# bergmanlab/TELR

Measured on AMD Instinct MI355X. Metric: gbp_aligned_per_s, higher is better.
Workload: dtype int16

## Files before the change

telr_amd/csrc/kernels.hip.h:

```cpp
#pragma once
#include <hip/hip_runtime.h>
#include <stdint.h>

#define TELR_NEG      (-(1 << 28))
#include "part_plan.h"
#define SK_TILE       1024
#define SK_THREADS    256
#define DP_DMAX       4096

struct ChainOpt {
    int32_t max_gap, bw, min_cnt, min_chain_score, chain_gap_q8, chain_skip_q8;
    int32_t dense_n, dense_span, mw_n;
};
struct DpOpt {
    int32_t a, b, q, e, q2, e2, sc_ambi, zdrop;
    int32_t cx_scale, cx_open, cx_emax, cx_emin, cx_dec, cx_flat;
};
__host__ __device__ __forceinline__ int d_cx_ext(const DpOpt &o, int len) { int v = o.cx_emax - o.cx_dec * len; return v > o.cx_emin ? v : o.cx_emin; }
__host__ __device__ __forceinline__ int d_cx_cost(const DpOpt &o, int L)
{
    int t = o.cx_open;
    for (int i = 0; i < L && i < o.cx_flat; ++i) t += d_cx_ext(o, i);
    if (L > o.cx_flat) t += (L - o.cx_flat) * o.cx_emin;
    return t;
// ... 1332 lines not shown
        for (int h = 1; h < R - 1; ++h) Ms = hfull[h] > Ms ? hfull[h] : Ms;
        Ms += (int32_t)sp1 + 1;
        const int inext = j0 + 64 + lane;
        const uint64_t knext = inext < n ? a[inext] : 0;
        const uint32_t ng = (uint32_t)(knext >> 32), nqp = (uint32_t)A_Q(knext), nsp1 = (uint32_t)A_SPAN(knext) - 1u;
        const int32_t nB = 2 * A_SPAN(knext) + 1;
        int32_t myB = 0, myp = -1;
        const int jn = n - j0 < 64 ? n - j0 : 64;
        for (int jj = 0; jj < jn; ++jj) {
            const int j = j0 + jj;
            const uint32_t gj = gcur, gj1 = gj + 1u;
            const uint32_t gnext = jj < 63 ? (uint32_t)__builtin_amdgcn_readlane((int)gi, jj + 1) : (uint32_t)__builtin_amdgcn_readlane((int)ng, 0);
            gcur = gnext;
            int32_t sB = __builtin_amdgcn_readlane(B, jj);
            const int32_t sMs = __builtin_amdgcn_readlane(Ms, jj);
            const bool me = lane == jj;
            if (sMs > (sB >> 1)) {
                const uint32_t gfar = jj ? (uint32_t)__builtin_amdgcn_readlane((int)hg[0], jj - 1) : (uint32_t)__builtin_amdgcn_readlane((int)hg[1], 63);
                if (gj - gfar <= max_gap) {
                    const uint32_t qS = (uint32_t)__builtin_amdgcn_readlane((int)qi, jj), spS = (uint32_t)__builtin_amdgcn_readlane((int)sp1, jj);
                    int32_t Bl = NEG * 2, bl = -1;
#pragma unroll
                    for (int h = R - 1; h >= 0; --h) {
                        const bool in_set = h == 0 ? lane < jj : h == R - 1 ? lane >= jj : true;
                        int32_t Bt = Bl, bt = bl;
                        d_chain_push<SKIP>(gj, qS, spS, hg[h] + 1u, hq[h] + 1u, hf[h], j0 - 64 * (h + 1) + lane, max_gap, ddc, gap_q8, skip_q8, Bt, bt);
                        Bl = in_set ? Bt : Bl; bl = in_set ? bt : bl;
                    }
                    int32_t m = Bl;
#pragma unroll
                    for (int s = 32; s >= 1; s >>= 1) { const int32_t v = __shfl_xor(m, s); m = v > m ? v : m; }
                    if (m > sB) {
                        int32_t w = Bl == m ? bl : -1;
#pragma unroll
                        for (int s = 32; s >= 1; s >>= 1) { const int32_t v = __shfl_xor(w, s); w = v > w ? v : w; }
                        B = me ? m : B; bp = me ? w : bp; sB = __builtin_amdgcn_readfirstlane(m);
                    }
                }
            }
            const uint32_t qj1 = (uint32_t)__builtin_amdgcn_readlane((int)qi, jj) + 1u;
            {
                const uint64_t one = 1ULL << jj; uint64_t sv;
                asm volatile("s_mov_b64 %[sv], exec\n\ts_mov_b64 exec, %[m]\n\t"
                             "v_mov_b32 %[myB], %[B]\n\tv_mov_b32 %[myp], %[bp]\n\tv_mov_b32 %[gi], %[ng]\n\tv_mov_b32 %[sp1], %[nsp1]\n\t"
                             "v_mov_b32 %[qi], %[nqp]\n\tv_mov_b32 %[B], %[nB]\n\ts_mov_b64 exec, %[sv]"
                             : [myB] "+v"(myB), [myp] "+v"(myp), [gi] "+v"(gi), [sp1] "+v"(sp1), [qi] "+v"(qi), [B] "+v"(B), [sv] "=&s"(sv)
                             : [bp] "v"(bp), [ng] "v"(ng), [nsp1] "v"(nsp1), [nqp] "v"(nqp), [nB] "v"(nB), [m] "s"(one));
            }
            if (gnext - gj <= max_gap) {
                const int32_t fj2p2 = (sB & ~1) + 2;
                d_chain_push<SKIP>(gi, qi, sp1, gj1, qj1, fj2p2, j, max_gap, ddc, gap_q8, skip_q8, B, bp);
            }
        }
        if (lane < jn) { f[base + j0 + lane] = myB >> 1; p[base + j0 + lane] = (myB & 1) ? -1 : myp + pdelta; }
        if (j0 + 64 < n) {
#pragma unroll
            for (int h = R - 1; h >= 1; --h) { hg[h] = hg[h - 1]; hq[h] = hq[h - 1]; hf[h] = hf[h - 1]; hsuf[h] = hsuf[h - 1]; hfull[h] = hfull[h - 1]; }
            const uint64_t k = a[j0 + lane];
            hg[0] = (uint32_t)(k >> 32); hq[0] = (uint32_t)A_Q(k); hf[0] = (myB & ~1) + 2;
            const int32_t fv = myB >> 1;
            int32_t inc = fv, suf = fv;
#pragma unroll
            for (int s = 1; s < 64; s <<= 1) {
                const int32_t u = __shfl_up(inc, s), d = __shfl_down(suf, s);
                if (lane >= s) inc = u > inc ? u : inc;
                if (lane + s < 64) suf = d > suf ? d : suf;
            }
            const int32_t ex = __shfl_up(inc, 1);
            pre0 = lane ? ex : NEG; hsuf[0] = suf; hfull[0] = __builtin_amdgcn_readlane(suf, 0);
        }
    }
}

__device__ __forceinline__ bool d_chain_dense(const uint64_t *__restrict__ a, const int n, const ChainOpt &o)
{
    if (o.dense_n <= 0 || n < o.dense_n || n < 128) return false;
    const int i = (int)(((int64_t)(threadIdx.x & 63) * (n - 65)) / 63);
    const uint32_t g0 = (uint32_t)(a[i] >> 32), g1 = (uint32_t)(a[i + 64] >> 32);
    return __popcll(__ballot(g1 - g0 <= (uint32_t)o.dense_span)) >= 21;
}
template <int R, bool SKIP>
__device__ __forceinline__ void d_chain_run_mw(const uint64_t *__restrict__ keys, const int64_t base, const int n, const int pdelta,
                                               const ChainOpt &o, int32_t *__restrict__ f, int32_t *__restrict__ p, uint4 *ring, int32_t *done_s)
{
    static_assert(R >= 2, "one wave is the push loop");
    constexpr int RING = 64 * R;
    const int lane = threadIdx.x & 63, wv = __builtin_amdgcn_readfirstlane((int)(threadIdx.x >> 6));
    const uint64_t *a = keys + base;
    const uint32_t max_gap = (uint32_t)o.max_gap, ddc = o.bw < o.max_gap ? (uint32_t)(o.max_gap - 1 - o.bw) : 0u;
    const uint32_t gap_q8 = (uint32_t)o.chain_gap_q8, skip_q8 = (uint32_t)o.chain_skip_q8;
    if (threadIdx.x == 0) *done_s = 0;
    __syncthreads();
    const int nchunk = (n + 63) >> 6;
    uint32_t gi, qi, sp1; int32_t B, bp = -1;
    { const int i = wv * 64 + lane; const uint64_t k = i < n ? a[i] : 0; gi = (uint32_t)(k >> 32); qi = (uint32_t)A_Q(k); sp1 = (uint32_t)A_SPAN(k) - 1u; B = 2 * A_SPAN(k) + 1; }
    for (int c = wv; c < nchunk; c += R) {
        const int j0 = c * 64;
        const int inext = j0 + RING + lane;
        const uint64_t knext = inext < n ? a[inext] : 0;
        const uint32_t ng = (uint32_t)(knext >> 32), nqp = (uint32_t)A_Q(knext), nsp1 = (uint32_t)A_SPAN(knext) - 1u;
        const int32_t nB = 2 * A_SPAN(knext) + 1;
        int j = j0 - 64 * (R - 1); if (j < 0) j = 0;
        int polls = 0;
        while (j < j0) {
            const int avail = __builtin_amdgcn_readfirstlane(__hip_atomic_load(done_s, __ATOMIC_ACQUIRE, __HIP_MEMORY_SCOPE_WORKGROUP));
            if (avail <= j) { if (++polls > (1 << 24)) break; __builtin_amdgcn_s_sleep(2); continue; }
            int lim = avail < j0 ? avail : j0; if (lim > j + 64) lim = j + 64;
            const int cnt = lim - j;
            uint4 e = make_uint4(0u, 0u, 0u, 0u);
            if (lane < cnt) e = ring[(j + lane) & (RING - 1)];
            for (int t = 0; t < cnt; ++t) {
                const uint32_t gj1 = (uint32_t)__builtin_amdgcn_readlane((int)e.x, t), qj1 = (uint32_t)__builtin_amdgcn_readlane((int)e.y, t);
                const int32_t fj2p2 = __builtin_amdgcn_readlane((int)e.z, t);
                d_chain_push<SKIP>(gi, qi, sp1, gj1, qj1, fj2p2, j + t, max_gap, ddc, gap_q8, skip_q8, B, bp);
            }
            j = lim;
        }
        const int jn = n - j0 < 64 ? n - j0 : 64;
        int32_t myB = 0, myp = -1; uint32_t myg = 0, myq = 0;
        for (int jj = 0; jj < jn; ++jj) {
            const uint32_t gj1 = (uint32_t)__builtin_amdgcn_readlane((int)gi, jj) + 1u, qj1 = (uint32_t)__builtin_amdgcn_readlane((int)qi, jj) + 1u;
            const int32_t fj2p2 = (__builtin_amdgcn_readlane(B, jj) & ~1) + 2;
            {
                const uint64_t one = 1ULL << jj; uint64_t sv;
                asm volatile("s_mov_b64 %[sv], exec\n\ts_mov_b64 exec, %[m]\n\t"
                             "v_mov_b32 %[myB], %[B]\n\tv_mov_b32 %[myp], %[bp]\n\tv_mov_b32 %[myg], %[gi]\n\tv_mov_b32 %[myq], %[qi]\n\t"
                             "v_mov_b32 %[gi], %[ng]\n\tv_mov_b32 %[qi], %[nqp]\n\tv_mov_b32 %[sp1], %[nsp1]\n\tv_mov_b32 %[B], %[nB]\n\ts_mov_b64 exec, %[sv]"
                             : [myB] "+v"(myB), [myp] "+v"(myp), [myg] "+v"(myg), [myq] "+v"(myq), [gi] "+v"(gi), [qi] "+v"(qi), [sp1] "+v"(sp1), [B] "+v"(B), [sv] "=&s"(sv)
                             : [bp] "v"(bp), [ng] "v"(ng), [nqp] "v"(nqp), [nsp1] "v"(nsp1), [nB] "v"(nB), [m] "s"(one));
            }
            d_chain_push<SKIP>(gi, qi, sp1, gj1, qj1, fj2p2, j0 + jj, max_gap, ddc, gap_q8, skip_q8, B, bp);
            if ((jj & 7) == 7 || jj == jn - 1) {
                if (lane >= (jj & ~7) && lane <= jj) ring[(j0 + lane) & (RING - 1)] = make_uint4(myg + 1u, myq + 1u, (uint32_t)((myB & ~1) + 2), 0u);
                __hip_atomic_store(done_s, j0 + jj + 1, __ATOMIC_RELEASE, __HIP_MEMORY_SCOPE_WORKGROUP);
            }
        }
        if (lane < jn) { f[base + j0 + lane] = myB >> 1; p[base + j0 + lane] = (myB & 1) ? -1 : myp + pdelta; }
    }
}
__device__ __forceinline__ bool d_chain_is_mw(const bool dense, const int n, const ChainOpt &o) { return dense && o.mw_n > 0 && n >= o.mw_n; }
template <int R, bool SKIP, int MODE>
__device__ __forceinline__ void d_chain_any(const uint64_t *__restrict__ keys, const int64_t base, const int n, const int pdelta,
                                            const ChainOpt &o, int32_t *__restrict__ f, int32_t *__restrict__ p, const bool skip_mw)
{
    if constexpr (MODE == 0 || R < 2) d_chain_run<R, SKIP>(keys, base, n, pdelta, o, f, p);
    else if constexpr (MODE == 1) d_chain_run_lazy<R, SKIP>(keys, base, n, pdelta, o, f, p);
    else {
        const bool dense = d_chain_dense(keys + base, n, o);
        if (skip_mw && d_chain_is_mw(dense, n, o)) return;
        if (dense) d_chain_run<R, SKIP>(keys, base, n, pdelta, o, f, p);
        else d_chain_run_lazy<R, SKIP>(keys, base, n, pdelta, o, f, p);
    }
}
template <int R, bool SKIP, int MODE = 2>
__global__ void __launch_bounds__(64) k_chain(const uint64_t *__restrict__ keys, const int32_t *__restrict__ q_aoff, int32_t nq,
                                              ChainOpt o, int32_t *__restrict__ f, int32_t *__restrict__ p, const int32_t *__restrict__ q_order, int32_t skip_mw)
{
    if ((int)blockIdx.x >= nq) return;
    const int q = q_order ? q_order[blockIdx.x] : blockIdx.x;
    d_chain_any<R, SKIP, MODE>(keys, q_aoff[q], q_aoff[q + 1] - q_aoff[q], 0, o, f, p, skip_mw != 0);
}
template <int R, bool SKIP>
__global__ void __launch_bounds__(64 * R) k_chain_mw(const uint64_t *__restrict__ keys, const int32_t *__restrict__ q_aoff, int32_t nq, const int32_t *__restrict__ list,
                                                     ChainOpt o, int32_t *__restrict__ f, int32_t *__restrict__ p)
{
    __shared__ uint4 ring[64 * R];
    __shared__ int32_t done_s;
    if ((int)blockIdx.x >= nq) return;
    const int q = list ? list[blockIdx.x] : (int)blockIdx.x;
    const int64_t base = q_aoff[q]; const int n = q_aoff[q + 1] - q_aoff[q];
    if (!d_chain_is_mw(d_chain_dense(keys + base, n, o), n, o)) return;
    d_chain_run_mw<R, SKIP>(keys, base, n, 0, o, f, p, ring, &done_s);
}
#define CHAIN_ISL_NQ 4096
__global__ void __launch_bounds__(256) k_isl_heads(const uint64_t *__restrict__ keys, const int32_t *__restrict__ q_aoff, int32_t nq, uint32_t max_gap, int32_t *__restrict__ head)
{
    const int q = blockIdx.x;
    if (q >= nq) return;
    const int64_t base = q_aoff[q]; const int n = q_aoff[q + 1] - q_aoff[q];
    for (int i = threadIdx.x; i < n; i += blockDim.x)
        head[base + i] = i == 0 || (uint32_t)(keys[base + i] >> 32) - (uint32_t)(keys[base + i - 1] >> 32) > max_gap;
}
__global__ void __launch_bounds__(256) k_isl_fill(const int32_t *__restrict__ q_aoff, int32_t nq, const int32_t *__restrict__ head, const int32_t *__restrict__ rank, int32_t na,
                                                  int32_t *__restrict__ isl_off, int32_t *__restrict__ isl_pd)
{
    const int q = blockIdx.x;
    if (q >= nq) return;
    const int64_t base = q_aoff[q]; const int n = q_aoff[q + 1] - q_aoff[q];
    for (int i = threadIdx.x; i < n; i += blockDim.x) if (head[base + i]) { const int id = rank[base + i]; isl_off[id] = (int32_t)base + i; isl_pd[id] = i; }
    if (q == 0 && threadIdx.x == 0) isl_off[rank[na]] = na;
}
template <int R, bool SKIP, int MODE = 2>
__global__ void __launch_bounds__(64) k_chain_isl(const uint64_t *__restrict__ keys, const int32_t *__restrict__ isl_off, const int32_t *__restrict__ isl_pd, const int32_t *__restrict__ nisl,
                                                  ChainOpt o, int32_t *__restrict__ f, int32_t *__restrict__ p)
{
    const int n_isl = *nisl;
    for (int s = blockIdx.x; s < n_isl; s += gridDim.x)
        d_chain_any<R, SKIP, MODE>(keys, isl_off[s], isl_off[s + 1] - isl_off[s], isl_pd[s], o, f, p, false);
}

#define CHAIN_SCAN_H    5000
#define CHAIN_SCAN_SKIP 25
__device__ __forceinline__ uint32_t d_wave_scan_max0(uint32_t v)
{
    v = max(v, (uint32_t)__builtin_amdgcn_update_dpp(0, (int)v, 0x111, 0xf, 0xf, true));
    v = max(v, (uint32_t)__builtin_amdgcn_update_dpp(0, (int)v, 0x112, 0xf, 0xf, true));
    v = max(v, (uint32_t)__builtin_amdgcn_update_dpp(0, (int)v, 0x114, 0xf, 0xf, true));
    v = max(v, (uint32_t)__builtin_amdgcn_update_dpp(0, (int)v, 0x118, 0xf, 0xf, true));
    v = max(v, (uint32_t)__builtin_amdgcn_update_dpp(0, (int)v, 0x142, 0xa, 0xf, true));
    v = max(v, (uint32_t)__builtin_amdgcn_update_dpp(0, (int)v, 0x143, 0xc, 0xf, true));
    return v;
}
template <bool SKIP>
__device__ __forceinline__ void d_chain_run_scan(const uint64_t *__restrict__ keys, const int64_t base, const int n, const int pdelta,
                                                 const ChainOpt &o, int32_t *__restrict__ f, int32_t *__restrict__ p, int32_t *__restrict__ mark,
                                                 uint8_t *__restrict__ fl)
{
    const int lane = threadIdx.x & 63;
    const uint64_t *a = keys + base;
    const uint32_t max_gap = (uint32_t)o.max_gap, ddc = o.bw < o.max_gap ? (uint32_t)(o.max_gap - 1 - o.bw) : 0u;
    const uint32_t gap_q8 = (uint32_t)o.chain_gap_q8, skip_q8 = (uint32_t)o.chain_skip_q8;
    uint32_t wg = 0, wq = 0; int32_t wf = 0, wp = -1;
    uint64_t kb = lane < n ? a[lane] : 0;
    for (int i0 = 0; i0 < n; i0 += 64) {
        const uint64_t kn = i0 + 64 + lane < n ? a[i0 + 64 + lane] : 0;
        const int m = n - i0 < 64 ? n - i0 : 64;
        int32_t of = 0, op = -1;
        for (int ii = 0; ii < m; ++ii) {
            const int i = i0 + ii;
            const uint32_t gi = (uint32_t)__builtin_amdgcn_readlane((int)(uint32_t)(kb >> 32), ii);
            const uint32_t klo = (uint32_t)__builtin_amdgcn_readlane((int)(uint32_t)kb, ii);
            const uint32_t qi = (klo >> 8) & 0xffffffu, sp = klo & 0xffu;
            const int32_t gpos = (int32_t)(gi & 0x7fffffffu);
            const int lo = i - CHAIN_SCAN_H > 0 ? i - CHAIN_SCAN_H : 0;
            int32_t best = (int32_t)sp, bp = -1, nskip = 0;
            for (int c = 0; ; ++c) {
                const int jt = i - 1 - 64 * c, j = jt - lane;
                if (jt < lo) break;
                uint32_t g = wg, q = wq; int32_t fj2p2 = wf, pj = wp; bool mk = false;
                if (c > 0 && j >= lo) {
                    const uint64_t k = a[j];
                    g = (uint32_t)(k >> 32); q = (uint32_t)A_Q(k);
                    fj2p2 = 2 * f[base + j] + 2;
                    const int32_t pa = p[base + j];
                    pj = pa >= 0 ? pa - pdelta : -1;
                    mk = mark[base + j] == (int32_t)(base + i);
                }
                const bool inw = j >= lo && ((g ^ gi) >> 31) == 0u && gpos - (int32_t)(g & 0x7fffffffu) <= (int32_t)max_gap;
                bool ok;
                const int32_t v2 = d_chain_link<SKIP>(gi, qi, sp - 1u, g + 1u, q + 1u, fj2p2, max_gap, ddc, gap_q8, skip_q8, ok);
                const bool valid = inw && ok;
                const int32_t v = v2 >> 1;
                const uint32_t u = valid && v > best ? (uint32_t)(v - best) : 0u;
                const uint32_t pre = d_wave_scan_max0(u);
                const uint32_t ex = (uint32_t)__shfl_up((int)pre, 1);
                const bool imp = u > (lane ? ex : 0u);
                fl[lane] = 0;
                const int tl = jt - pj;
                if (valid && pj >= 0 && tl < 64) fl[tl] = 1;
                __builtin_amdgcn_fence(__ATOMIC_SEQ_CST, "wavefront");
                mk = mk || fl[lane] != 0;
                __builtin_amdgcn_fence(__ATOMIC_SEQ_CST, "wavefront");
                const int32_t s = valid ? (imp ? -1 : (mk ? 1 : 0)) : 0;
                const int32_t T = nskip + (int32_t)d_wave_scan_add((uint32_t)s);
                const int32_t x = T + (int32_t)d_wave_scan_max0(T < 0 ? (uint32_t)(-T) : 0u);
                const uint64_t brk = __ballot(x > CHAIN_SCAN_SKIP);
                const int b = brk ? __ffsll((unsigned long long)brk) - 1 : 64;
                const uint64_t scanned = b == 64 ? ~0ULL : ((1ULL << b) - 1);
                const uint64_t im = __ballot(imp) & scanned;
                if (im) {
                    const int hl = 63 - __clzll((long long)im);
                    best += (int32_t)__builtin_amdgcn_readlane((int)u, hl);
                    bp = jt - hl;
                }
                const uint64_t win = __ballot(inw);
                const bool more = b == 64 && win == ~0ULL && jt - 64 >= lo;
                if (!more) break;
                if (valid && pj >= 0 && tl >= 64) mark[base + pj] = (int32_t)(base + i);
                nskip = __builtin_amdgcn_readlane(x, 63);
                __threadfence_block();
            }
            of = lane == ii ? best : of; op = lane == ii ? bp : op;
            wg = (uint32_t)__shfl_up((int)wg, 1); wq = (uint32_t)__shfl_up((int)wq, 1); wf = __shfl_up(wf, 1); wp = __shfl_up(wp, 1);
            if (lane == 0) { wg = gi; wq = qi; wf = 2 * best + 2; wp = bp; }
        }
        if (lane < m) {
            f[base + i0 + lane] = of; p[base + i0 + lane] = op >= 0 ? op + pdelta : -1;
            mark[base + i0 + lane] = -1;
        }
        __threadfence_block();
        kb = kn;
    }
}
template <bool SKIP>
__global__ void __launch_bounds__(64) k_chain_scan(const uint64_t *__restrict__ keys, const int32_t *__restrict__ q_aoff, int32_t nq,
                                                   ChainOpt o, int32_t *__restrict__ f, int32_t *__restrict__ p, int32_t *__restrict__ mark,
                                                   const int32_t *__restrict__ q_order)
{
    __shared__ uint8_t fl[64];
    if ((int)blockIdx.x >= nq) return;
    const int q = q_order ? q_order[blockIdx.x] : blockIdx.x;
    d_chain_run_scan<SKIP>(keys, q_aoff[q], q_aoff[q + 1] - q_aoff[q], 0, o, f, p, mark, fl);
}
template <bool SKIP>
__global__ void __launch_bounds__(64) k_chain_scan_isl(const uint64_t *__restrict__ keys, const int32_t *__restrict__ isl_off, const int32_t *__restrict__ isl_pd,
                                                       const int32_t *__restrict__ nisl, ChainOpt o, int32_t *__restrict__ f, int32_t *__restrict__ p,
                                                       int32_t *__restrict__ mark)
{
    __shared__ uint8_t fl[64];
    const int n_isl = *nisl;
    for (int s = blockIdx.x; s < n_isl; s += gridDim.x)
        d_chain_run_scan<SKIP>(keys, isl_off[s], isl_off[s + 1] - isl_off[s], isl_pd[s], o, f, p, mark, fl);
}
// ... 2148 lines not shown
```

telr_amd/csrc/telr_engine.hip:

```cpp
#include <hip/hip_runtime.h>
#include <cstring>
#include <string.h>
#include <rocprim/rocprim.hpp>
#include <algorithm>
#include <atomic>
#include <immintrin.h>
#include <chrono>
#include <cmath>
#include <condition_variable>
#include <cstdio>
#include <cstdlib>
#include <cstring>
#include <map>
#include <memory>
#include <mutex>
#include <string>
#include <thread>
#include <sys/mman.h>
#include <vector>
#include "../../include/telr_hip.h"
#include "kernels.hip.h"
#include "range_plan.h"
#include "sam_records.h"
#define TELR_HAVE_SEED_ARGS 1
// ... 1344 lines not shown
        hipLaunchKernelGGL(k_tb_scatter, dim3(np / 256 + 1), dim3(256), 0, st, d_probs, d_clslist, np, coff, d_tboff);
        HIPCHK(hipGetLastError());
        HIPCHK(hipMemcpyAsync(&tb_total, d_tboff + np, 8, hipMemcpyDeviceToHost, st));
        HIPCHK(hipStreamSynchronize(st));
    }
    uint8_t *d_tb;
    TRY(ctx_buf_t(ctx, ("tb" + sfx).c_str(), (size_t)tb_total + 256, &d_tb));
    if (primary) TRY(ctx_buf_t(ctx, "rawcig", (size_t)cg_total + 16, d_rawcig_io));
    DpArgs D; D.qseq2 = qs->d_seq2; D.qnmask = qs->d_nmask; D.tseq2 = tg->d_seq2; D.tnmask = tg->d_nmask; D.probs = d_probs;
    D.qtot = qs->padded_bases; D.ttot = tg->padded_bases;
    D.o.a = mo->a; D.o.b = mo->b; D.o.q = mo->q; D.o.e = mo->e; D.o.q2 = mo->q2; D.o.e2 = mo->e2; D.o.sc_ambi = mo->sc_ambi; D.o.zdrop = mo->zdrop;
    D.o.cx_scale = D.o.cx_open = D.o.cx_emax = D.o.cx_emin = D.o.cx_dec = D.o.cx_flat = 0;
    if (mo->cx_scale > 0) {
        const int S = mo->cx_scale;
        D.o.a *= S; D.o.b *= S; D.o.sc_ambi *= S; D.o.zdrop *= S;
        D.o.cx_scale = S; D.o.cx_open = mo->cx_open; D.o.cx_emax = mo->cx_ext_max; D.o.cx_emin = mo->cx_ext_min; D.o.cx_dec = mo->cx_decay;
        D.o.cx_flat = mo->cx_decay > 0 && mo->cx_ext_max > mo->cx_ext_min ? (mo->cx_ext_max - mo->cx_ext_min + mo->cx_decay - 1) / mo->cx_decay : 0;
    }
    D.tb = d_tb; D.cig = *d_rawcig_io; D.res = d_res; D.dcap = 0;
    D.retry = d_retry; D.tb4 = L.tb4_mask; D.tag8_steps = L.tag8_steps;
    static const bool tb_split = !ab_on("tb_one_launch");
    int nw = 0; uint32_t *d_wv2 = nullptr;
    {
        PkPlan plan; plan.woff[0] = 0;
        for (int c = 0; c < PK_NC; ++c) { const int ppw = 64 / DP_CLASS[PK_CLS(c)].lpp; plan.woff[c + 1] = plan.woff[c] + (h_cls[PK_CLS(c)] + ppw - 1) / ppw; }
        nw = plan.woff[PK_NC];
        if (nw > 0) {
            uint32_t *d_wk, *d_wv, *d_wk2;
            TRY(ctx_buf_t(ctx, ("pk_wkey" + sfx).c_str(), (size_t)nw, &d_wk));
            TRY(ctx_buf_t(ctx, ("pk_wval" + sfx).c_str(), (size_t)nw, &d_wv));
            TRY(ctx_buf_t(ctx, ("pk_wkey2" + sfx).c_str(), (size_t)nw, &d_wk2));
            TRY(ctx_buf_t(ctx, ("pk_wval2" + sfx).c_str(), (size_t)nw, &d_wv2));
            hipLaunchKernelGGL(k_pk_waves, dim3((nw + 255) / 256), dim3(256), 0, st, d_probs, d_clslist, coff, plan, d_wk, d_wv);
            HIPCHK(hipGetLastError());
            size_t tbytes = 0;
            HIPCHK(rocprim::radix_sort_pairs_desc(nullptr, tbytes, d_wk, d_wk2, d_wv, d_wv2, (size_t)nw, 0, 16, st));
            void *tmp; TRY(ctx_buf(ctx, "rp_tmp", tbytes, &tmp));
            HIPCHK(rocprim::radix_sort_pairs_desc(tmp, tbytes, d_wk, d_wk2, d_wv, d_wv2, (size_t)nw, 0, 16, st));
        }
    }
    HIPCHK(hipEventRecord(ctx->ev_fork, st));
    int side = 0;
    std::vector<hipStream_t> used;
    static const bool serial = getenv("TELR_SERIAL") != nullptr;
    auto side_stream = [&]() { if (serial) return st; hipStream_t s2 = ctx->side[side % TELR_NSIDE]; ++side; used.push_back(s2); return s2; };
    auto launch = [&](int c, DpKernel kernel, hipStream_t s2) -> int {
        const int nl = h_cls[c];
        int threads = DP_CLASS[c].lpp > 64 ? DP_CLASS[c].lpp : 64, ppb = DP_CLASS[c].lpp < 64 ? 64 / DP_CLASS[c].lpp : 1;
        size_t lds = 0;
        D.list = d_clslist + coff.off[c]; D.nlist = nl; D.dcap = 0;
        if (DP_CLASS[c].family == DPF_LDS) {
            D.dcap = DP_CLASS[c].maxd;
            lds = (size_t)(D.dcap + 2) * 5 * 4;
            static const bool one_wave = ab_on("dp_one_wave");
            if (one_wave) { kernel = k_dp; threads = 64; }
            if (lds > 48 * 1024) HIPCHK(hipFuncSetAttribute((const void*)kernel, hipFuncAttributeMaxDynamicSharedMemorySize, (int)lds));
        }
        if (c == CLS_PKX64 && nl < 8192) { kernel = k_dp_pkx16; ppb = 4; }
        hipLaunchKernelGGL(kernel, dim3((nl + ppb - 1) / ppb), dim3(threads), lds, s2, D);
        HIPCHK(hipGetLastError());
        return TELR_OK;
    };
    for (const SideLaunch &row : SIDE_LAUNCH) {
        const int c = row.cls, nl = h_cls[c];
        if (nl == 0) continue;
        hipStream_t s2 = side_stream();
        HIPCHK(hipStreamWaitEvent(s2, ctx->ev_fork, 0));
        TRY(launch(c, row.kernel, s2));
        if (tb_split) {
            const int tbw_max = 2048;
            if (row.lane_walk || nl > tbw_max) hipLaunchKernelGGL(k_traceback, dim3((nl + 63) / 64), dim3(64), 0, s2, d_probs, d_res, nl, d_tb, *d_rawcig_io, d_retry, D.list);
            else hipLaunchKernelGGL(k_traceback_w, dim3(nl), dim3(64), 0, s2, d_probs, d_res, nl, d_tb, *d_rawcig_io, d_retry, D.list);
            HIPCHK(hipGetLastError());
        }
    }
    D.dcap = 0;
    const bool tb_over = tb_split && !serial && nw > 0;
    if (primary) HIPCHK(hipEventRecord(ctx->evk[5], st));
    if (primary && nw > 0) ++ctx->pk_launches;
    if (nw > 0) {
        D.list = nullptr; D.nlist = 0;
        if (tb_over) { HIPCHK(hipStreamWaitEvent(ctx->tb_stream, ctx->ev_fork, 0)); if (primary) HIPCHK(hipEventRecord(ctx->evk[3], ctx->tb_stream)); }
        hipLaunchKernelGGL(k_dp_pk, dim3(nw), dim3(64), 0, st, D, d_wv2, d_clslist, coff);
        HIPCHK(hipGetLastError());
        if (tb_over) {
            HIPCHK(hipEventRecord(ctx->ev_pk, st));
            HIPCHK(hipStreamWaitEvent(ctx->tb_stream, ctx->ev_pk, 0));
            hipLaunchKernelGGL(k_traceback_pk, dim3(nw), dim3(64), 0, ctx->tb_stream, d_probs, d_res, d_tb, *d_rawcig_io, d_retry, d_wv2, d_clslist, coff, L.tb4_mask, D.o, L.tag8_steps);
            HIPCHK(hipGetLastError());
            if (primary) HIPCHK(hipEventRecord(ctx->evk[4], ctx->tb_stream));
            used.push_back(ctx->tb_stream);
        }
    }
    if (primary) HIPCHK(hipEventRecord(ctx->evk[0], st));
    if (h_cls[CLS_REG64]) TRY(launch(CLS_REG64, reg_kernel<CLS_REG64>(), st));
    if (h_cls[CLS_REG128]) TRY(launch(CLS_REG128, reg_kernel<CLS_REG128>(), st));
    if (primary) HIPCHK(hipEventRecord(ctx->evk[1], st));
    if (tb_split) {
        if (!tb_over && primary) HIPCHK(hipEventRecord(ctx->evk[3], st));
        if (!tb_over && nw > 0) hipLaunchKernelGGL(k_traceback_pk, dim3(nw), dim3(64), 0, st, d_probs, d_res, d_tb, *d_rawcig_io, d_retry, d_wv2, d_clslist, coff, L.tb4_mask, D.o, L.tag8_steps);
        for (int c : { (int)CLS_REG128, (int)CLS_REG64 }) {
            if (h_cls[c] == 0) continue;
            hipLaunchKernelGGL(k_traceback, dim3((h_cls[c] + 63) / 64), dim3(64), 0, st, d_probs, d_res, h_cls[c], d_tb, *d_rawcig_io, d_retry, (const int32_t*)(d_clslist + coff.off[c]));
        }
        if (!tb_over && primary) HIPCHK(hipEventRecord(ctx->evk[4], st));
        HIPCHK(hipGetLastError());
    }
    for (size_t u = 0; u < used.size(); ++u) {
        HIPCHK(hipEventRecord(ctx->ev_side[u % TELR_NSIDE], used[u]));
        HIPCHK(hipStreamWaitEvent(st, ctx->ev_side[u % TELR_NSIDE], 0));
    }
#ifdef TB_PROF
    if (nw > 0) {
        HIPCHK(hipDeviceSynchronize());
        unsigned long long h[8]; HIPCHK(hipMemcpyFromSymbol(h, HIP_SYMBOL(g_tb_prof), sizeof(h)));
        unsigned long long z[8] = {0, 0, 0, 0, ~0ULL, 0, 0, 0}; HIPCHK(hipMemcpyToSymbol(HIP_SYMBOL(g_tb_prof), z, sizeof(z)));
        if (h[2]) fprintf(stderr, "[tb prof] k_traceback_pk: %llu waves, span %.3f ms, longest wave %.3f ms (%llu lines), mean wave %.3f ms, %.1f lines per wave, wave-ms / span = %.1f waves on the device on average\n",
                          h[2], (double)(h[5] - h[4]) / 1e5, (double)(h[1] >> 16) / 1e5, h[1] & 0xffffULL, (double)h[0] / (double)h[2] / 1e5, (double)h[3] / (double)h[2], (double)h[0] / (double)(h[5] - h[4] ? h[5] - h[4] : 1));
    }
#endif
    if (!tb_split) {
        if (primary) HIPCHK(hipEventRecord(ctx->evk[3], st));
        hipLaunchKernelGGL(k_traceback, dim3((np + 63) / 64), dim3(64), 0, st, d_probs, d_res, np, d_tb, *d_rawcig_io, d_retry, (const int32_t*)nullptr);
        if (primary) HIPCHK(hipEventRecord(ctx->evk[4], st));
    }
    HIPCHK(hipGetLastError());
    return TELR_OK;
}

struct HostTrace {
    bool on; const char *tag; std::chrono::steady_clock::time_point t0, last;
    HostTrace(const char *t) : tag(t) { static const bool e = trace_on("host"); on = e; t0 = last = std::chrono::steady_clock::now(); }
    void mark(const char *what) {
        if (!on) return;
        auto now = std::chrono::steady_clock::now();
        fprintf(stderr, "[host %s] %-28s +%7.3f ms  (%8.3f)\n", tag, what, std::chrono::duration<double, std::milli>(now - last).count(), std::chrono::duration<double, std::milli>(now - t0).count());
        last = now;
    }
};

struct OccCut { int32_t mid_occ; const int32_t *d_tmid; };
static int chain_dispatch(telr_ctx *ctx, hipStream_t st, const telr_map_opt *mo, const uint64_t *d_skeys, const int32_t *d_qaoff, int nq, int32_t na,
                          int32_t n_over, const int32_t *d_overlist, const int32_t *d_qorder, int32_t *d_f, int32_t *d_p)
{
    ChainOpt co; co.max_gap = mo->max_gap; co.bw = mo->bw_long > mo->bw ? mo->bw_long : mo->bw; co.min_cnt = mo->min_cnt; co.min_chain_score = mo->min_chain_score;
    co.chain_gap_q8 = mo->chain_gap_q8; co.chain_skip_q8 = mo->chain_skip_q8;
    static const bool chain_push = ab_on("chain_push"), chain_lazy = ab_on("chain_lazy"), chain_no_mw = ab_on("chain_no_mw");
    static int dense_v[3] = {2048, 48, 1 << 19};
    static const bool dense_env = [] { if (const char *e = getenv("TELR_CHAIN_DENSE")) sscanf(e, "%d%*[,:]%d%*[,:]%d", &dense_v[0], &dense_v[1], &dense_v[2]); return true; }();
    (void)dense_env;
    const int Rr = mo->chain_lookback / 64;
    const bool mw_all = dense_v[2] <= SEGSORT_CAP;
    static const bool no_islands = ab_on("no_islands");
    const bool islands = nq <= CHAIN_ISL_NQ && na > 0 && !no_islands;
    const bool mw = !(mo->flags & TELR_MF_CHAIN_SKIP) && !chain_push && !chain_lazy && !chain_no_mw && Rr >= 2 && na > 0 && !islands && dense_v[2] > 0 && (mw_all || n_over > 0);
    co.dense_n = dense_v[0]; co.dense_span = dense_v[1]; co.mw_n = mw ? dense_v[2] : 0;
#define CHAIN_LAUNCH(RR, SK) do { if (chain_push) hipLaunchKernelGGL((k_chain<RR, SK, 0>), dim3(nq), dim3(64), 0, st, d_skeys, d_qaoff, nq, co, d_f, d_p, d_qorder, 0); \
                                  else if (chain_lazy) hipLaunchKernelGGL((k_chain<RR, SK, 1>), dim3(nq), dim3(64), 0, st, d_skeys, d_qaoff, nq, co, d_f, d_p, d_qorder, 0); \
                                  else hipLaunchKernelGGL((k_chain<RR, SK, 2>), dim3(nq), dim3(64), 0, st, d_skeys, d_qaoff, nq, co, d_f, d_p, d_qorder, mw ? 1 : 0); } while (0)
#define CHAIN_MW(RR, SK) hipLaunchKernelGGL((k_chain_mw<RR, SK>), dim3(mw_all ? nq : n_over), dim3(64 * RR), 0, ctx->side[0], d_skeys, d_qaoff, mw_all ? nq : n_over, mw_all ? (const int32_t*)nullptr : (const int32_t*)d_overlist, co, d_f, d_p)
    const bool skip = co.chain_skip_q8 != 0;
    if (mo->flags & TELR_MF_CHAIN_SKIP) {
        int32_t *d_mark;
        TRY(ctx_buf_t(ctx, "chain_mark", (size_t)na + 1, &d_mark));
        if (islands) {
            int32_t *d_head, *d_rank, *d_ioff, *d_ipd;
            TRY(ctx_buf_t(ctx, "isl_head", (size_t)na + 1, &d_head));
            TRY(ctx_buf_t(ctx, "isl_rank", (size_t)na + 1, &d_rank));
            TRY(ctx_buf_t(ctx, "isl_off", (size_t)na + 2, &d_ioff));
            TRY(ctx_buf_t(ctx, "isl_pd", (size_t)na + 1, &d_ipd));
            HIPCHK(hipMemsetAsync(d_head + na, 0, 4, st));
            hipLaunchKernelGGL(k_isl_heads, dim3(nq), dim3(256), 0, st, d_skeys, d_qaoff, nq, (uint32_t)co.max_gap, d_head);
            HIPCHK(hipGetLastError());
            TRY((dev_exclusive_scan<int32_t, int32_t>(ctx, d_head, d_rank, (size_t)na + 1)));
            hipLaunchKernelGGL(k_isl_fill, dim3(nq), dim3(256), 0, st, d_qaoff, nq, d_head, d_rank, (int32_t)na, d_ioff, d_ipd);
            const unsigned grid = (unsigned)std::min<int64_t>((int64_t)na, 256 * 32);
            if (skip) hipLaunchKernelGGL(k_chain_scan_isl<true>, dim3(grid), dim3(64), 0, st, d_skeys, d_ioff, d_ipd, d_rank + na, co, d_f, d_p, d_mark);
            else hipLaunchKernelGGL(k_chain_scan_isl<false>, dim3(grid), dim3(64), 0, st, d_skeys, d_ioff, d_ipd, d_rank + na, co, d_f, d_p, d_mark);
        } else if (nq > 0) {
            if (skip) hipLaunchKernelGGL(k_chain_scan<true>, dim3(nq), dim3(64), 0, st, d_skeys, d_qaoff, nq, co, d_f, d_p, d_mark, d_qorder);
            else hipLaunchKernelGGL(k_chain_scan<false>, dim3(nq), dim3(64), 0, st, d_skeys, d_qaoff, nq, co, d_f, d_p, d_mark, d_qorder);
        }
        HIPCHK(hipGetLastError());
        return TELR_OK;
    }
    if (islands) {
        int32_t *d_head, *d_rank, *d_ioff, *d_ipd;
        TRY(ctx_buf_t(ctx, "isl_head", (size_t)na + 1, &d_head));
        TRY(ctx_buf_t(ctx, "isl_rank", (size_t)na + 1, &d_rank));
        TRY(ctx_buf_t(ctx, "isl_off", (size_t)na + 2, &d_ioff));
        TRY(ctx_buf_t(ctx, "isl_pd", (size_t)na + 1, &d_ipd));
        HIPCHK(hipMemsetAsync(d_head + na, 0, 4, st));
        hipLaunchKernelGGL(k_isl_heads, dim3(nq), dim3(256), 0, st, d_skeys, d_qaoff, nq, (uint32_t)co.max_gap, d_head);
        HIPCHK(hipGetLastError());
        TRY((dev_exclusive_scan<int32_t, int32_t>(ctx, d_head, d_rank, (size_t)na + 1)));
        hipLaunchKernelGGL(k_isl_fill, dim3(nq), dim3(256), 0, st, d_qaoff, nq, d_head, d_rank, (int32_t)na, d_ioff, d_ipd);
        const unsigned grid = (unsigned)std::min<int64_t>((int64_t)na, 256 * 32);
#define CHAIN_ISL(RR, SK) do { if (chain_push) hipLaunchKernelGGL((k_chain_isl<RR, SK, 0>), dim3(grid), dim3(64), 0, st, d_skeys, d_ioff, d_ipd, d_rank + na, co, d_f, d_p); \
                               else if (chain_lazy) hipLaunchKernelGGL((k_chain_isl<RR, SK, 1>), dim3(grid), dim3(64), 0, st, d_skeys, d_ioff, d_ipd, d_rank + na, co, d_f, d_p); \
                               else hipLaunchKernelGGL((k_chain_isl<RR, SK, 2>), dim3(grid), dim3(64), 0, st, d_skeys, d_ioff, d_ipd, d_rank + na, co, d_f, d_p); } while (0)
        if (Rr == 1) { if (skip) CHAIN_ISL(1, true); else CHAIN_ISL(1, false); }
        else if (Rr == 2) { if (skip) CHAIN_ISL(2, true); else CHAIN_ISL(2, false); }
        else { if (skip) CHAIN_ISL(4, true); else CHAIN_ISL(4, false); }
#undef CHAIN_ISL
    }
    else {
        if (mw) {
            HIPCHK(hipEventRecord(ctx->ev_side[0], st));
            HIPCHK(hipStreamWaitEvent(ctx->side[0], ctx->ev_side[0], 0));
            if (Rr == 2) { if (skip) CHAIN_MW(2, true); else CHAIN_MW(2, false); }
            else { if (skip) CHAIN_MW(4, true); else CHAIN_MW(4, false); }
            HIPCHK(hipEventRecord(ctx->ev_side[0], ctx->side[0]));
        }
        if (Rr == 1) { if (skip) CHAIN_LAUNCH(1, true); else CHAIN_LAUNCH(1, false); }
        else if (Rr == 2) { if (skip) CHAIN_LAUNCH(2, true); else CHAIN_LAUNCH(2, false); }
        else { if (skip) CHAIN_LAUNCH(4, true); else CHAIN_LAUNCH(4, false); }
        if (mw) HIPCHK(hipStreamWaitEvent(st, ctx->ev_side[0], 0));
    }
#undef CHAIN_LAUNCH
#undef CHAIN_MW
    HIPCHK(hipGetLastError());
    return TELR_OK;
}

struct BtOut { uint64_t *d_canch; int32_t *d_choff, *d_nch; ChainRec *d_rec; int32_t npk_tot; };
static int backtrack_dispatch(telr_ctx *ctx, hipStream_t st, const telr_map_opt *mo, const uint64_t *d_skeys, const int32_t *d_qaoff, int nq, int32_t na,
                              bool any_over, const int32_t *d_qorder, const int32_t *d_f, const int32_t *d_p, BtOut *out)
{
    uint8_t *d_flags; uint64_t *d_pk, *d_pk2, *d_canch; int32_t *d_npk, *d_pkend, *d_choff, *d_nch;
    TRY(ctx_buf_t(ctx, "flags", (size_t)na + 16, &d_flags));
    uint8_t *d_nonpeak = d_flags;
    TRY(ctx_buf_t(ctx, "pk", (size_t)na, &d_pk));
    TRY(ctx_buf_t(ctx, "pk2", (size_t)na, &d_pk2));
    TRY(ctx_buf_t(ctx, "canch", (size_t)na, &d_canch));
    TRY(ctx_buf_t(ctx, "n_peaks", (size_t)nq + 1, &d_npk));
    TRY(ctx_buf_t(ctx, "pk_end", (size_t)nq + 1, &d_pkend));
    TRY(ctx_buf_t(ctx, "ch_off", (size_t)nq + 1, &d_choff));
    TRY(ctx_buf_t(ctx, "n_chains", (size_t)nq + 1, &d_nch));
    HIPCHK(hipMemsetAsync(d_flags, 0, (size_t)na + 16, st));
    hipLaunchKernelGGL(k_nonpeak, dim3(nq), dim3(256), 0, st, d_qaoff, d_f, d_p, d_nonpeak);
    hipLaunchKernelGGL(k_peaks, dim3(nq), dim3(256), 0, st, d_qaoff, d_f, d_nonpeak, mo->min_chain_score, d_pk, d_npk, d_pkend);
    HIPCHK(hipGetLastError());
    if (na > 0) TRY(seg_sort_u64(ctx, "so_p", d_pk, d_pk2, d_qaoff, d_pkend, nullptr, d_qorder, nq, (size_t)na, any_over, st));
    HIPCHK(hipMemsetAsync(d_npk + nq, 0, 4, st));
    TRY((dev_exclusive_scan<int32_t, int32_t>(ctx, d_npk, d_choff, (size_t)nq + 1)));
    int32_t npk_tot = 0;
    HIPCHK(hipMemcpyAsync(&npk_tot, d_choff + nq, 4, hipMemcpyDeviceToHost, st));
    HIPCHK(hipStreamSynchronize(st));
    ChainRec *d_rec;
    TRY(ctx_buf_t(ctx, "chain_rec", (size_t)npk_tot, &d_rec));
    {
        uint32_t *d_owner; int32_t *d_depth, *d_chtop, *d_chaoff;
        TRY(ctx_buf_t(ctx, "bt_owner", (size_t)na + 1, &d_owner));
        TRY(ctx_buf_t(ctx, "bt_depth", (size_t)na + 1, &d_depth));
        TRY(ctx_buf_t(ctx, "bt_chtop", (size_t)na + 1, &d_chtop));
        TRY(ctx_buf_t(ctx, "bt_chaoff", (size_t)na + 1, &d_chaoff));
        HIPCHK(hipMemsetAsync(d_owner, 0xff, ((size_t)na + 1) * 4, st));
        hipLaunchKernelGGL(k_bt_rank, dim3(nq), dim3(256), 0, st, d_qaoff, d_pk2, d_npk, d_owner);
        if (mo->flags & TELR_MF_CHAIN_SKIP) {
            hipLaunchKernelGGL(k_bt_owner<BT_RING_SCAN>, dim3(nq), dim3(64), 0, st, d_qaoff, nq, d_p, (int32_t)CHAIN_SCAN_H, d_owner, d_qorder);
            hipLaunchKernelGGL(k_bt_depth<BT_RING_SCAN>, dim3(nq), dim3(64), 0, st, d_qaoff, nq, d_p, d_owner, d_depth, d_chtop, d_qorder);
        } else {
            hipLaunchKernelGGL(k_bt_owner<BT_RING>, dim3(nq), dim3(64), 0, st, d_qaoff, nq, d_p, mo->chain_lookback, d_owner, d_qorder);
            hipLaunchKernelGGL(k_bt_depth<BT_RING>, dim3(nq), dim3(64), 0, st, d_qaoff, nq, d_p, d_owner, d_depth, d_chtop, d_qorder);
        }
        hipLaunchKernelGGL(k_bt_emit, dim3(nq), dim3(64), 0, st, d_skeys, d_qaoff, nq, d_f, d_p, d_pk2, d_npk, d_choff, mo->min_chain_score, mo->min_cnt,
                           d_owner, d_depth, d_chtop, d_chaoff, d_rec, d_nch, d_qorder);
        hipLaunchKernelGGL(k_bt_scatter, dim3(nq), dim3(256), 0, st, d_skeys, d_qaoff, d_owner, d_depth, d_chaoff, d_canch, d_qorder);
        HIPCHK(hipGetLastError());
    }
    HIPCHK(hipGetLastError());
    out->d_canch = d_canch; out->d_choff = d_choff; out->d_nch = d_nch; out->d_rec = d_rec; out->npk_tot = npk_tot;
    return TELR_OK;
}

struct SelOut { int nk; KeptLite *hl; KeptChain *d_kc; const uint64_t *d_sk2; const uint8_t *d_keep; };
static int select1_dispatch(telr_ctx *ctx, hipStream_t st, const telr_map_opt *mo, const int32_t *d_choff, const int32_t *d_nch, const ChainRec *d_rec, int32_t npk_tot,
                            const int32_t *d_qaoff, int nq, int32_t q0, const int32_t *d_qlen, const int64_t *d_qboff, const uint32_t *d_goff, const int32_t *d_tlen,
                            const int64_t *d_tboff, int32_t n_targets, bool any_over, const int32_t *d_qorder, bool need_recs, int32_t *h_nch, int32_t *q_k0, SelOut *out)
{
    uint64_t *d_sk, *d_sk2; int32_t *d_segend, *d_pfs, *d_pfe, *d_ptid, *d_pkey, *d_tct, *d_tcn, *d_nkept, *d_koff; uint8_t *d_keep;
    TRY(ctx_buf_t(ctx, "sel_key", (size_t)npk_tot + 1, &d_sk));
    TRY(ctx_buf_t(ctx, "sel_key2", (size_t)npk_tot + 1, &d_sk2));
    TRY(ctx_buf_t(ctx, "sel_segend", (size_t)nq + 1, &d_segend));
    TRY(ctx_buf_t(ctx, "sel_pfs", (size_t)npk_tot + 1, &d_pfs));
    TRY(ctx_buf_t(ctx, "sel_pfe", (size_t)npk_tot + 1, &d_pfe));
    TRY(ctx_buf_t(ctx, "sel_ptid", (size_t)npk_tot + 1, &d_ptid));
    TRY(ctx_buf_t(ctx, "sel_pkey", (size_t)npk_tot + 1, &d_pkey));
    TRY(ctx_buf_t(ctx, "sel_tct", (size_t)npk_tot + 1, &d_tct));
    TRY(ctx_buf_t(ctx, "sel_tcn", (size_t)npk_tot + 1, &d_tcn));
    TRY(ctx_buf_t(ctx, "sel_keep", (size_t)npk_tot + 1, &d_keep));
    TRY(ctx_buf_t(ctx, "sel_nkept", (size_t)nq + 2, &d_nkept));
    TRY(ctx_buf_t(ctx, "sel_koff", (size_t)nq + 2, &d_koff));
    hipLaunchKernelGGL(k_sel_keys, dim3(nq), dim3(64), 0, st, d_choff, d_nch, d_rec, d_sk, d_segend);
    HIPCHK(hipGetLastError());
    if (npk_tot > 0) TRY(seg_sort_u64(ctx, "so_c", d_sk, d_sk2, d_choff, d_segend, nullptr, d_qorder, nq, (size_t)npk_tot, any_over, st));
    SelOpt so; so.mask_level = mo->mask_level; so.pri_ratio = mo->pri_ratio; so.best_n = mo->best_n; so.secondary = mo->secondary;
    so.per_target = (mo->flags & TELR_MF_PER_TARGET) ? 1 : 0;
    hipLaunchKernelGGL(k_select1, dim3(nq), dim3(64), 0, st, d_choff, d_nch, d_rec, d_sk2, d_qlen, d_goff, n_targets, so,
                       d_pfs, d_pfe, d_ptid, d_pkey, d_tct, d_tcn, d_keep, d_nkept, d_qorder);
    HIPCHK(hipGetLastError());
    HIPCHK(hipMemsetAsync(d_nkept + nq, 0, 4, st));
    TRY((dev_exclusive_scan<int32_t, int32_t>(ctx, d_nkept, d_koff, (size_t)nq + 1)));
    HIPCHK(hipMemcpyAsync(q_k0, d_koff, (size_t)(nq + 1) * 4, hipMemcpyDeviceToHost, st));
    if (!need_recs) HIPCHK(hipMemcpyAsync(h_nch, d_nch, (size_t)nq * 4, hipMemcpyDeviceToHost, st));
    HIPCHK(hipStreamSynchronize(st));
    const int nk = q_k0[nq];
    KeptLite *d_kl;
    KeptChain *d_kc; KeptLite *hl;
    TRY(ctx_buf_t(ctx, "kept", (size_t)nk, &d_kc));
    TRY(ctx_buf_t(ctx, "kept_lite", (size_t)nk, &d_kl));
    TRY(ctx_hbuf_t(ctx, "h_kept_lite", (size_t)nk, &hl));
// ... 1163 lines not shown
```

Baseline: 21.66.

## Split chaining at max-gap islands and batch small islands in one wavefront

The per-query chain kernel now walks each anchor list in segments separated by gaps larger than max_gap. Up to 64 anchors that fall in complete islands are chained in one wavefront pass using ballot and ds_bpermute lane exchange. Larger islands are located by scanning ahead with ballots and handed to the existing dense/lazy chain routine with a position offset. The aim is to stop paying full lookback chaining cost over anchors that cannot link across large gaps, at the price of extra scan passes and a new code path that can be turned off with an A/B flag.

```diff
diff --git a/telr_amd/csrc/kernels.hip.h b/telr_amd/csrc/kernels.hip.h
--- a/telr_amd/csrc/kernels.hip.h
+++ b/telr_amd/csrc/kernels.hip.h
@@ -1508,13 +1508,77 @@
         else d_chain_run_lazy<R, SKIP>(keys, base, n, pdelta, o, f, p);
     }
 }
+template <int R, bool SKIP>
+__device__ __forceinline__ void d_chain_walk(const uint64_t *__restrict__ keys, const int64_t base, const int n,
+                                             const ChainOpt &o, int32_t *__restrict__ f, int32_t *__restrict__ p, const bool pack)
+{
+    const int lane = threadIdx.x & 63;
+    const uint64_t *a = keys + base;
+    const uint32_t max_gap = (uint32_t)o.max_gap, ddc = o.bw < o.max_gap ? (uint32_t)(o.max_gap - 1 - o.bw) : 0u;
+    const uint32_t gap_q8 = (uint32_t)o.chain_gap_q8, skip_q8 = (uint32_t)o.chain_skip_q8;
+    const uint64_t upto = (2ULL << lane) - 1ULL;
+    const int lane4 = lane << 2;
+    int pos = 0;
+    while (pos < n) {
+        int end = n;
+        if (pack) {
+            const int i = pos + lane;
+            const uint64_t k = i < n ? a[i] : 0;
+            const uint32_t gi = (uint32_t)(k >> 32);
+            const uint32_t gprev = (uint32_t)__shfl_up((int)gi, 1);
+            const uint64_t heads = __ballot(i < n && gi - gprev > max_gap) | 1ULL;
+            int e = n - pos;
+            if (e > 64) { const uint64_t hh = heads & ~1ULL; e = hh ? 63 - __clzll((long long)hh) : 0; }
+            if (e > 0) {
+                const uint32_t qi = (uint32_t)A_Q(k), sp1 = (uint32_t)A_SPAN(k) - 1u;
+                int32_t B = 2 * A_SPAN(k) + 1, bp4 = 0;
+                int src4 = lane < e ? (63 - __clzll((long long)(heads & upto))) << 2 : lane4;
+                for (;;) {
+                    const bool act = src4 < lane4;
+                    if (__ballot(act) == 0) break;
+                    const uint32_t gj1 = (uint32_t)__builtin_amdgcn_ds_bpermute(src4, (int)gi) + 1u;
+                    const uint32_t qj1 = (uint32_t)__builtin_amdgcn_ds_bpermute(src4, (int)qi) + 1u;
+                    const int32_t fj2p2 = (__builtin_amdgcn_ds_bpermute(src4, B) & ~1) + 2;
+                    bool ok;
+                    const int32_t v2 = d_chain_link<SKIP>(gi, qi, sp1, gj1, qj1, fj2p2, max_gap, ddc, gap_q8, skip_q8, ok);
+                    if (act && ok && v2 >= B) { B = v2; bp4 = src4; }
+                    src4 += 4;
+                }
+                if (lane < e) { f[base + i] = B >> 1; p[base + i] = (B & 1) ? -1 : pos + (bp4 >> 2); }
+                pos += e;
+                continue;
+            }
+            for (int c = pos + 64; c < n; c += 256) {
+                uint64_t hm[4];
+#pragma unroll
+                for (int u = 0; u < 4; ++u) {
+                    const int ii = c + 64 * u + lane;
+                    bool h = false;
+                    if (ii < n) h = (uint32_t)(a[ii] >> 32) - (uint32_t)(a[ii - 1] >> 32) > max_gap;
+                    hm[u] = __ballot(h);
+                }
+                int at = -1;
+#pragma unroll
+                for (int u = 3; u >= 0; --u) if (hm[u]) at = c + 64 * u + __ffsll((long long)hm[u]) - 1;
+                if (at >= 0) { end = at; break; }
+            }
+        }
+        d_chain_any<R, SKIP, 2>(keys, base + pos, end - pos, pos, o, f, p, false);
+        pos = end;
+    }
+}
 template <int R, bool SKIP, int MODE = 2>
 __global__ void __launch_bounds__(64) k_chain(const uint64_t *__restrict__ keys, const int32_t *__restrict__ q_aoff, int32_t nq,
-                                              ChainOpt o, int32_t *__restrict__ f, int32_t *__restrict__ p, const int32_t *__restrict__ q_order, int32_t skip_mw)
+                                              ChainOpt o, int32_t *__restrict__ f, int32_t *__restrict__ p, const int32_t *__restrict__ q_order, int32_t skip_mw, int32_t pack)
 {
     if ((int)blockIdx.x >= nq) return;
     const int q = q_order ? q_order[blockIdx.x] : blockIdx.x;
-    d_chain_any<R, SKIP, MODE>(keys, q_aoff[q], q_aoff[q + 1] - q_aoff[q], 0, o, f, p, skip_mw != 0);
+    const int64_t base = q_aoff[q]; const int n = q_aoff[q + 1] - q_aoff[q];
+    if constexpr (MODE != 2) d_chain_any<R, SKIP, MODE>(keys, base, n, 0, o, f, p, false);
+    else {
+        if (skip_mw && d_chain_is_mw(d_chain_dense(keys + base, n, o), n, o)) return;
+        d_chain_walk<R, SKIP>(keys, base, n, o, f, p, pack != 0);
+    }
 }
 template <int R, bool SKIP>
 __global__ void __launch_bounds__(64 * R) k_chain_mw(const uint64_t *__restrict__ keys, const int32_t *__restrict__ q_aoff, int32_t nq, const int32_t *__restrict__ list,
diff --git a/telr_amd/csrc/telr_engine.hip b/telr_amd/csrc/telr_engine.hip
--- a/telr_amd/csrc/telr_engine.hip
+++ b/telr_amd/csrc/telr_engine.hip
@@ -1520,12 +1520,13 @@
     const int Rr = mo->chain_lookback / 64;
     const bool mw_all = dense_v[2] <= SEGSORT_CAP;
     static const bool no_islands = ab_on("no_islands");
+    static const bool chain_no_pack = ab_on("chain_no_pack");
     const bool islands = nq <= CHAIN_ISL_NQ && na > 0 && !no_islands;
     const bool mw = !(mo->flags & TELR_MF_CHAIN_SKIP) && !chain_push && !chain_lazy && !chain_no_mw && Rr >= 2 && na > 0 && !islands && dense_v[2] > 0 && (mw_all || n_over > 0);
     co.dense_n = dense_v[0]; co.dense_span = dense_v[1]; co.mw_n = mw ? dense_v[2] : 0;
-#define CHAIN_LAUNCH(RR, SK) do { if (chain_push) hipLaunchKernelGGL((k_chain<RR, SK, 0>), dim3(nq), dim3(64), 0, st, d_skeys, d_qaoff, nq, co, d_f, d_p, d_qorder, 0); \
-                                  else if (chain_lazy) hipLaunchKernelGGL((k_chain<RR, SK, 1>), dim3(nq), dim3(64), 0, st, d_skeys, d_qaoff, nq, co, d_f, d_p, d_qorder, 0); \
-                                  else hipLaunchKernelGGL((k_chain<RR, SK, 2>), dim3(nq), dim3(64), 0, st, d_skeys, d_qaoff, nq, co, d_f, d_p, d_qorder, mw ? 1 : 0); } while (0)
+#define CHAIN_LAUNCH(RR, SK) do { if (chain_push) hipLaunchKernelGGL((k_chain<RR, SK, 0>), dim3(nq), dim3(64), 0, st, d_skeys, d_qaoff, nq, co, d_f, d_p, d_qorder, 0, 0); \
+                                  else if (chain_lazy) hipLaunchKernelGGL((k_chain<RR, SK, 1>), dim3(nq), dim3(64), 0, st, d_skeys, d_qaoff, nq, co, d_f, d_p, d_qorder, 0, 0); \
+                                  else hipLaunchKernelGGL((k_chain<RR, SK, 2>), dim3(nq), dim3(64), 0, st, d_skeys, d_qaoff, nq, co, d_f, d_p, d_qorder, mw ? 1 : 0, chain_no_pack ? 0 : 1); } while (0)
 #define CHAIN_MW(RR, SK) hipLaunchKernelGGL((k_chain_mw<RR, SK>), dim3(mw_all ? nq : n_over), dim3(64 * RR), 0, ctx->side[0], d_skeys, d_qaoff, mw_all ? nq : n_over, mw_all ? (const int32_t*)nullptr : (const int32_t*)d_overlist, co, d_f, d_p)
     const bool skip = co.chain_skip_q8 != 0;
     if (mo->flags & TELR_MF_CHAIN_SKIP) {
```

New measurement: 23.27, median of 6. 1.07x the previous value.
